# JBLanier/stratego_env

Hardware: AMD Instinct MI355X
Metric: env steps/sec (higher is better)
Workload: dtype u8

## Files before the change

stratego_env_amd/csrc/sgx_layout.h:

```cpp
#pragma once

namespace {

constexpr int OBS_CH = SGX_PO_OBS_CHANNELS;
constexpr int LUT_STRIDE = SGX_OBS_LUT_STRIDE;
constexpr int FOBS_CH = SGX_FO_OBS_CHANNELS;
constexpr int LUT_ROW_PITCH = 33, LUT_BLK = 673 , LUT_DWORDS = 2 * LUT_BLK + 2;
#ifndef SGX_WPB
#define SGX_WPB 8
#endif
#ifndef SGX_MIN_WAVES
#define SGX_MIN_WAVES 6
#endif
constexpr int QTAB_DWORDS = 2 * OBS_CH * 4, OBS_TAB_DWORDS = LUT_DWORDS + QTAB_DWORDS;
constexpr int FOBS_TAB_DWORDS = LUT_DWORDS + 2 * FOBS_CH * 4;
constexpr int NIB_ONE = 4, CODE_NONE = 0xFF, CODETAB_REC = 192, CODETAB_BYTES = 208;
constexpr int COMBAT_BYTES = 16 * 16;
enum { COMBAT_LOSE = 0, COMBAT_TIE = 1, COMBAT_WIN = 2, COMBAT_WIN_FLAG = 3 };
__host__ __device__ inline int combat_outcome(int att, int def) {
    if (att == 3  && def == 12 ) return COMBAT_WIN;
    if (att == 1  && def == 10 ) return COMBAT_WIN;
    if (def == 11 ) return COMBAT_WIN_FLAG;
    if (def == 12) return COMBAT_LOSE;
    if (att == def) return COMBAT_TIE;
// ... 168 lines not shown
    z ^= z >> 30; z *= 0xBF58476D1CE4E5B9ull;
    z ^= z >> 27; z *= 0x94D049BB133111EBull;
    z ^= z >> 31;
    return z;
}
__host__ __device__ inline uint64_t sgx_rng(uint64_t seed, uint64_t g, uint64_t j, uint32_t stream, uint32_t t) {
    uint64_t h = sm_fin(seed + 0x9E3779B97F4A7C15ull * (g + 1));
    uint64_t ctr = ((uint64_t)stream << 32) | t;
    return sm_fin(h ^ (j * 0xD1B54A32D192ED03ull + ctr * 0x8CB92BA72F3D8DD7ull + 0x2545F4914F6CDD1Dull));
}
__host__ __device__ inline uint32_t rng_below(uint64_t r, uint32_t n) { return (uint32_t)(((r >> 32) * (uint64_t)n) >> 32); }
enum { STREAM_SETUP = 0, STREAM_ACTION = 1, STREAM_SHUFFLE_P1 = 2, STREAM_SHUFFLE_P2 = 3, STREAM_POOL = 4, STREAM_DETERMINIZE = 5 };
__host__ __device__ inline int pool_index(uint64_t seed, uint64_t g, uint64_t j, int n_pool) {
    return (int)rng_below(sgx_rng(seed, g, j, STREAM_POOL, 0), (uint32_t)n_pool);
}
__host__ __device__ inline int pool_first_player(uint64_t seed, uint64_t g, uint64_t j, int pool_flags) {
    if (!(pool_flags & SGX_POOL_RANDOM_FIRST_PLAYER)) return 0;
    return rng_below(sgx_rng(seed, g, j, STREAM_POOL, 1), 2u) == 1u ? -1 : 1;
}

template <class G>
__device__ inline int4 *rec_scal(int8_t *boards, int rec_bytes, int64_t env) {
    return reinterpret_cast<int4 *>(boards + env * (int64_t)rec_bytes + G::SC_OFF);
}

template <class G, class KP>
__device__ inline int max_events_of(const KP &P) { return G::BIG ? (int)G::EVL_MAX : P.max_events; }

template <class G>
__device__ inline int uni(int x) {
    if constexpr (G::LPG == 64) return __builtin_amdgcn_readfirstlane(x);
    else return x;
}
template <class G>
__device__ inline unsigned long long gballot(bool pred) {
    const unsigned long long b = __ballot(pred);
    if constexpr (G::LPG == 64) return b;
    else return (b >> (__lane_id() & ~(G::LPG - 1))) & ((1ull << G::LPG) - 1ull);
}

template <int CTRL, int ROW_MASK = 0xF>
__device__ inline int dpp_or_zero(int x) { return __builtin_amdgcn_update_dpp(0, x, CTRL, ROW_MASK, 0xF, true); }
template <class G>
__device__ inline int gscan_incl(int x) {
    x += dpp_or_zero<0x111>(x);
    x += dpp_or_zero<0x112>(x);
    x += dpp_or_zero<0x114>(x);
    x += dpp_or_zero<0x118>(x);
    if constexpr (G::LPG >= 32) x += dpp_or_zero<0x142, 0xA>(x);
    if constexpr (G::LPG == 64) x += dpp_or_zero<0x143, 0xC>(x);
    return x;
}
template <class G>
__device__ inline int glane(int x, int l) {
    if constexpr (G::LPG == 64) return __builtin_amdgcn_readlane(x, __builtin_amdgcn_readfirstlane(l));
    else return __shfl(x, l, G::LPG);
}
__device__ inline int quad_sum(int x) {
    x += __builtin_amdgcn_update_dpp(0, x, 0xB1, 0xF, 0xF, true);
    x += __builtin_amdgcn_update_dpp(0, x, 0x4E, 0xF, 0xF, true);
    return x;
}

template <class KP>
__device__ inline int64_t group_of_block(const KP &P) {
    const int64_t nb = gridDim.x, b = blockIdx.x;
    const int x = (int)(b & 7);
    const int64_t i = b >> 3;
    if (P.map_mode == 0) {
        if (i >= P.xcd_count[x]) return (int64_t)1 << 40;
        return P.xcd_first[x] + i;
    }
    const int64_t per = nb >> 3;
    const int map_arg = P.map_arg;
    if (P.map_mode == 1) return b;
    if (P.map_mode == 2) { const int64_t s = map_arg; return (i / s) * (8 * s) + x * s + (i % s); }
    if (P.map_mode == 3) return x * per + (i + x * (int64_t)map_arg) % per;
    if (P.map_mode == 4) return x * per + (per - 1 - i);
    if (P.map_mode == 5) return x * per + ((x & 1) ? per - 1 - i : i);
    if (P.map_mode == 6) { const int64_t f = map_arg, sub = per / f; return x * per + (i % f) * sub + (i / f); }
    return x * per + i;
}

template <class G>
__device__ inline void wave_sync() {
    __builtin_amdgcn_fence(__ATOMIC_RELEASE, "wavefront");
    __builtin_amdgcn_wave_barrier();
    __builtin_amdgcn_fence(__ATOMIC_ACQUIRE, "wavefront");
}

struct PartialObs {
    static constexpr int NCH = OBS_CH;
    static constexpr bool CODES = true;
    static constexpr int OWN0 = 0, ENEMY0 = -1 , OWN_PO0 = 12, ENEMY_PO0 = 25, OBST = 38, REC0 = 39, CAP0 = 41,
                         STILL0 = 65;
};
struct FullObs {
    static constexpr int NCH = FOBS_CH;
    static constexpr bool CODES = true;
    static constexpr int OWN0 = 0, ENEMY0 = 12, OWN_PO0 = 24, ENEMY_PO0 = 37, OBST = 50, REC0 = 51, CAP0 = 53, STILL0 = 77;
};
struct OrigPartialObs {
    static constexpr int NCH = SGX_PO_OBS_CHANNELS_ORIGINAL;
    static constexpr bool CODES = false;
    static constexpr int REC0 = 4, CAP0 = 6;
    __device__ static inline int board(int ch, int qi) {
        if (ch == 0) return B_PIECES + qi;
        if (ch == 1) return B_PO + qi;
        if (ch == 2) return B_PO + (1 - qi);
        if (ch == 3) return B_OBST;
        if (ch == 4) return B_RECENT + qi;
        if (ch == 5) return B_RECENT + (1 - qi);
        if (ch < 30) return B_ZERO;
        if (ch == 30) return B_STILL + qi;
        return B_STILL + (1 - qi);
    }
    __device__ static inline int bias(int ch) { return (ch == 4 || ch == 5) ? 3 : 0; }
};
struct OrigFullObs {
    static constexpr int NCH = SGX_FO_OBS_CHANNELS_ORIGINAL;
    static constexpr bool CODES = false;
    static constexpr int REC0 = 3, CAP0 = 7;
    __device__ static inline int board(int ch, int qi) {
        if (ch == 0) return B_PIECES + qi;
        if (ch == 1) return B_PIECES + (1 - qi);
        if (ch == 2) return B_OBST;
        if (ch == 3) return B_RECENT + qi;
        if (ch == 4) return B_RECENT + (1 - qi);
        if (ch == 5) return B_PO + qi;
        if (ch == 6) return B_PO + (1 - qi);
        if (ch < 31) return B_ZERO;
        if (ch == 31) return B_STILL + qi;
        return B_STILL + (1 - qi);
    }
    __device__ static inline int bias(int ch) { return (ch == 3 || ch == 4) ? 3 : 0; }
};
template <int KIND>
struct ObsKind {
    static constexpr bool FULL = (KIND & 1) != 0, ORIG = (KIND & 2) != 0, NOOBS = (KIND & 8) != 0;
    static_assert(!NOOBS || KIND == 8, "the no-observation kind stands alone");
    static constexpr int NIB_CH = (ORIG || NOOBS) ? 0 : (FULL ? FOBS_CH : OBS_CH);
    using P = std::conditional_t<ORIG, OrigPartialObs, PartialObs>;
    using F = std::conditional_t<ORIG, OrigFullObs, FullObs>;
};

}
```

stratego_env_amd/csrc/sgx_step.h:

```cpp
#pragma once

namespace {

template <class G, int KIND>
constexpr int tmpl_bytes(bool full) { return ((G::RC * (full ? FOBS_CH : OBS_CH) + 1) / 2 + 15) & ~15; }
template <class G, int KIND>
constexpr int tmpl_lds_bytes(bool full) { return G::WIDE ? 0 : tmpl_bytes<G, KIND>(full); }
template <class G, int KIND>
constexpr int shared_table_bytes() {
    constexpr bool FULL = (KIND & 1) != 0, ORIG = (KIND & 2) != 0;
    if (ObsKind<KIND>::NOOBS) return 16;
    if (ORIG) return 4 * (OBS_TAB_DWORDS + (FULL ? FOBS_TAB_DWORDS : 0));
    return tmpl_lds_bytes<G, KIND>(false) + (FULL ? tmpl_lds_bytes<G, KIND>(true) : 0) + CODETAB_BYTES;
}

template <class G, int KIND, bool MAPPED = false>
constexpr int waves_per_simd() {
    constexpr int per_wg = G::WPB * G::GPW * (int)sizeof(Lds<G, ObsKind<KIND>::NIB_CH>) + shared_table_bytes<G, KIND>() + G::OBST_BYTES + COMBAT_BYTES;
    constexpr int wgs = (160 * 1024) / per_wg;
    constexpr int w = wgs * G::WPB / 4;
    constexpr int want = (G::HALF || (MAPPED && ObsKind<KIND>::NOOBS)) ? 6 : (G::RC <= 64 ? 8 : SGX_MIN_WAVES);
    return w > want ? want : (w < 1 ? 1 : w);
}

// ... 568 lines not shown
        const int na = kth_valid(L, (int)k, lane);
        if constexpr (PERSIST) {
            carry->na = na;
            if (lane == 0 && P.traj_act_log) P.traj_act_log[env + (int64_t)carry->slot * P.traj_out_envs] = na;
        }
        if (lane == 0 && (!PERSIST || last)) P.io.next_actions_dev[env] = na;
    }

    STAMP(7);
    bool dirty = applied || wrote_reset || (MAPPED && P.src_boards);
    if constexpr (PERSIST) {
        dirty = dirty || (!first && carry->dirty);
        carry->turn = turn; carry->flags = flags; carry->game_no = game_no; carry->max_turns = max_turns;
        carry->n_events = n_events; carry->rp0 = rp0; carry->rp1 = rp1; carry->dirty = dirty;
        if (!last) dirty = false;
    }
    if (dirty)
        write_record(L, rec_g, G::BIG ? (int)G::IMG_BYTES : P.rec_bytes, make_int4(turn, flags, max_turns, game_no), make_int4(n_events, rp0, rp1, 0), n_events, lane);
    STAMP(8);
#ifdef SGX_STAMPS
    asm volatile("s_waitcnt vmcnt(0)" ::: "memory");
    STAMP(9);
#endif
}

template <int R_, int C_, int KIND, bool MAPPED, int VAR = 0>
__device__ __forceinline__ void game_kernel_body(const KParams &P) {
    using G = Geo<R_, C_, VAR>;
    static_assert(VAR == 0 || (VAR == 2 && ObsKind<KIND>::NOOBS), "two games per wave: the no-observation kinds only");
    using PS = typename ObsKind<KIND>::P;
    using FS = typename ObsKind<KIND>::F;
    constexpr bool FULL = ObsKind<KIND>::FULL, ORIG = ObsKind<KIND>::ORIG;
    __shared__ Lds<G, ObsKind<KIND>::NIB_CH> LW[G::WPB * G::GPW];
    __shared__ alignas(16) uint8_t shared[shared_table_bytes<G, KIND>()];
    __shared__ alignas(16) uint8_t obst_s[G::OBST_BYTES + COMBAT_BYTES];
    const int lane = threadIdx.x & (G::LPG - 1), slot = threadIdx.x / G::LPG;
    const int64_t env = P.env_first + group_of_block(P) * (G::WPB * G::GPW) + slot;
    const GameInput in = load_game<G, MAPPED>(P, env, lane);
    const bool raw = (P.io.flags & SGX_STEP_RAW_OBS) != 0;
    if constexpr (ObsKind<KIND>::NOOBS) {
    } else if constexpr (ORIG) {
        float *lut_s = reinterpret_cast<float *>(shared);
        const f32x4 *lsrc = reinterpret_cast<const f32x4 *>(P.tab->lut[4 + (raw ? 2 : 0)]);
        for (int i = threadIdx.x; i < LUT_DWORDS / 4; i += 64 * G::WPB) reinterpret_cast<f32x4 *>(lut_s)[i] = lsrc[i];
        build_quad_table<G, PS>(reinterpret_cast<uint32_t *>(lut_s + LUT_DWORDS), threadIdx.x, 64 * G::WPB);
        if constexpr (FULL) {
            const f32x4 *fsrc = reinterpret_cast<const f32x4 *>(P.tab->lut[4 + (raw ? 2 : 0) + 1]);
            for (int i = threadIdx.x; i < LUT_DWORDS / 4; i += 64 * G::WPB) reinterpret_cast<f32x4 *>(lut_s + OBS_TAB_DWORDS)[i] = fsrc[i];
            build_quad_table<G, FS>(reinterpret_cast<uint32_t *>(lut_s + OBS_TAB_DWORDS + LUT_DWORDS), threadIdx.x, 64 * G::WPB);
        }
    } else {
        constexpr int NP = tmpl_lds_bytes<G, KIND>(false), NF = FULL ? tmpl_lds_bytes<G, KIND>(true) : 0;
        const int4 *tp = reinterpret_cast<const int4 *>(P.tab->tmpl[raw ? 2 : 0]);
        for (int i = threadIdx.x; i < NP / 16; i += 64 * G::WPB) reinterpret_cast<int4 *>(shared)[i] = tp[i];
        if constexpr (FULL) {
            const int4 *tf = reinterpret_cast<const int4 *>(P.tab->tmpl[(raw ? 2 : 0) + 1]);
            for (int i = threadIdx.x; i < NF / 16; i += 64 * G::WPB) reinterpret_cast<int4 *>(shared + NP)[i] = tf[i];
        }
        const int4 *ct = reinterpret_cast<const int4 *>(P.tab->codetab[raw ? 1 : 0]);
        for (int i = threadIdx.x; i < CODETAB_BYTES / 16; i += 64 * G::WPB) reinterpret_cast<int4 *>(shared + NP + NF)[i] = ct[i];
    }
    for (int i = threadIdx.x; i < G::S / 4; i += 64 * G::WPB) reinterpret_cast<int *>(obst_s)[i] = reinterpret_cast<const int *>(P.tab->obstacles)[i];
    for (int i = threadIdx.x; i < COMBAT_BYTES / 4; i += 64 * G::WPB)
        reinterpret_cast<int *>(obst_s + G::OBST_BYTES)[i] = reinterpret_cast<const int *>(P.tab->combat)[i];
    __syncthreads();
    if (env < P.n_envs) env_step<R_, C_, KIND, MAPPED, false, VAR>(P, LW[slot], shared, obst_s, env, lane, in);
}

template <int R_, int C_, int KIND, bool MAPPED = false, int VAR = 0>
__global__ __launch_bounds__((64 * Geo<R_, C_, VAR>::WPB), (waves_per_simd<Geo<R_, C_, VAR>, KIND, MAPPED>())) void step_kernel(const KParams P) {
    game_kernel_body<R_, C_, KIND, MAPPED, VAR>(P);
}
template <int R_, int C_, int KIND, bool MAPPED = false, int VAR = 0>
__global__ __launch_bounds__((64 * Geo<R_, C_, VAR>::WPB), (waves_per_simd<Geo<R_, C_, VAR>, KIND, MAPPED>())) void observe_kernel(const KParams P) {
    game_kernel_body<R_, C_, KIND, MAPPED, VAR>(P);
}

constexpr int WSTEPS_MAX_SETS = 8;
struct WaveStepsParams {
    KParams k;
    int32_t n_steps, n_sets, first_set;
    int32_t strided;
    int32_t barrier;
    int64_t obs_slot_bytes, fobs_slot_bytes, mask_slot_bytes;
    float *const *obs_tab, *const *fobs_tab;
    uint8_t *const *mask_tab;
    float *obs[WSTEPS_MAX_SETS], *fobs[WSTEPS_MAX_SETS];
    uint8_t *mask[WSTEPS_MAX_SETS];
};
template <class SPP>
__device__ __forceinline__ void steps_outputs_of(const SPP sp, const int set, StepCarry &carry) {
    if (sp->strided == 2) {
        carry.obs = table_entry(sp->obs_tab, set);
        carry.fobs = table_entry(sp->fobs_tab, set);
        carry.mask = table_entry(sp->mask_tab, set);
    } else if (sp->strided) {
        carry.obs = reinterpret_cast<float *>(reinterpret_cast<char *>(sp->obs[0]) + (int64_t)set * sp->obs_slot_bytes);
        carry.fobs = reinterpret_cast<float *>(reinterpret_cast<char *>(sp->fobs[0]) + (int64_t)set * sp->fobs_slot_bytes);
        carry.mask = sp->mask[0] + (int64_t)set * sp->mask_slot_bytes;
    } else {
        carry.obs = sp->obs[set];
        carry.fobs = sp->fobs[set];
        carry.mask = sp->mask[set];
    }
    carry.slot = set;
}
template <class G, int KIND>
constexpr int steps_waves_per_simd() {
    constexpr int w = waves_per_simd<G, KIND, false>();
    return (G::RC <= 64 && G::RC % 4 != 0 && !ObsKind<KIND>::NOOBS && w > 6) ? 6 : w;
}
struct WaveStepsParamsPool {
    WaveStepsParams w;
    PoolParams pool;
};
__device__ __forceinline__ const SGX_KERNARG WaveStepsParams *wsp_of(const SGX_KERNARG WaveStepsParams *p) { return p; }
__device__ __forceinline__ const SGX_KERNARG WaveStepsParams *wsp_of(const SGX_KERNARG WaveStepsParamsPool *p) { return &p->w; }
template <int R_, int C_, int KIND, int VAR, class SPT = WaveStepsParamsPool>
__device__ __forceinline__ void steps_body(const SPT &SP) {
    constexpr bool POOL = true;
    using G = Geo<R_, C_, VAR>;
    static_assert(VAR == 0 || (VAR == 2 && ObsKind<KIND>::NOOBS), "two games per wave: the no-observation kinds only");
    using PS = typename ObsKind<KIND>::P;
    using FS = typename ObsKind<KIND>::F;
    constexpr bool FULL = ObsKind<KIND>::FULL, ORIG = ObsKind<KIND>::ORIG;
#if defined(__HIP_DEVICE_COMPILE__)
    const SGX_KERNARG SPT *top = (const SGX_KERNARG SPT *)__builtin_amdgcn_kernarg_segment_ptr();
#else
    const SPT *top = &SP;
#endif
    const SGX_KERNARG WaveStepsParams *spp = wsp_of(top);
    const SGX_KERNARG KParams &P = spp->k;
    __shared__ Lds<G, ObsKind<KIND>::NIB_CH> LW[G::WPB * G::GPW];
    __shared__ alignas(16) uint8_t shared[shared_table_bytes<G, KIND>()];
    __shared__ alignas(16) uint8_t obst_s[G::OBST_BYTES + COMBAT_BYTES];
    const int lane = threadIdx.x & (G::LPG - 1), slot = threadIdx.x / G::LPG;
    const int64_t env = P.env_first + group_of_block(P) * (G::WPB * G::GPW) + slot;
    const GameInput in = load_game<G, false>(P, env, lane);
    const bool raw = (P.io.flags & SGX_STEP_RAW_OBS) != 0;
    if constexpr (ObsKind<KIND>::NOOBS) {
    } else if constexpr (ORIG) {
        float *lut_s = reinterpret_cast<float *>(shared);
        const f32x4 *lsrc = reinterpret_cast<const f32x4 *>(P.tab->lut[4 + (raw ? 2 : 0)]);
        for (int i = threadIdx.x; i < LUT_DWORDS / 4; i += 64 * G::WPB) reinterpret_cast<f32x4 *>(lut_s)[i] = lsrc[i];
        build_quad_table<G, PS>(reinterpret_cast<uint32_t *>(lut_s + LUT_DWORDS), threadIdx.x, 64 * G::WPB);
        if constexpr (FULL) {
            const f32x4 *fsrc = reinterpret_cast<const f32x4 *>(P.tab->lut[4 + (raw ? 2 : 0) + 1]);
            for (int i = threadIdx.x; i < LUT_DWORDS / 4; i += 64 * G::WPB) reinterpret_cast<f32x4 *>(lut_s + OBS_TAB_DWORDS)[i] = fsrc[i];
            build_quad_table<G, FS>(reinterpret_cast<uint32_t *>(lut_s + OBS_TAB_DWORDS + LUT_DWORDS), threadIdx.x, 64 * G::WPB);
        }
    } else {
        constexpr int NP = tmpl_lds_bytes<G, KIND>(false), NF = FULL ? tmpl_lds_bytes<G, KIND>(true) : 0;
        const int4 *tp = reinterpret_cast<const int4 *>(P.tab->tmpl[raw ? 2 : 0]);
        for (int i = threadIdx.x; i < NP / 16; i += 64 * G::WPB) reinterpret_cast<int4 *>(shared)[i] = tp[i];
        if constexpr (FULL) {
            const int4 *tf = reinterpret_cast<const int4 *>(P.tab->tmpl[(raw ? 2 : 0) + 1]);
            for (int i = threadIdx.x; i < NF / 16; i += 64 * G::WPB) reinterpret_cast<int4 *>(shared + NP)[i] = tf[i];
        }
        const int4 *ct = reinterpret_cast<const int4 *>(P.tab->codetab[raw ? 1 : 0]);
        for (int i = threadIdx.x; i < CODETAB_BYTES / 16; i += 64 * G::WPB) reinterpret_cast<int4 *>(shared + NP + NF)[i] = ct[i];
    }
    for (int i = threadIdx.x; i < G::S / 4; i += 64 * G::WPB) reinterpret_cast<int *>(obst_s)[i] = reinterpret_cast<const int *>(P.tab->obstacles)[i];
    for (int i = threadIdx.x; i < COMBAT_BYTES / 4; i += 64 * G::WPB)
        reinterpret_cast<int *>(obst_s + G::OBST_BYTES)[i] = reinterpret_cast<const int *>(P.tab->combat)[i];
    __syncthreads();
    if (env >= P.n_envs) return;
    int set = spp->first_set;
    const int n_steps = spp->n_steps;
    if constexpr (POOL) {
        StepCarryPool carry{};
        for (int t = 0; t < n_steps; ++t) {
            const SGX_KERNARG SPT *tp = top;
            int lane_t = lane, slot_t = slot;
            asm volatile("" : "+s"(tp), "+v"(lane_t), "+v"(slot_t));
            const SGX_KERNARG WaveStepsParams *sp = wsp_of(tp);
            if (t && sp->barrier) __builtin_amdgcn_s_barrier();
            steps_outputs_of(sp, set, carry);
            carry.first = t == 0;
            env_step<R_, C_, KIND, false, false, VAR, 3, true>(sp->k, LW[slot_t], shared, obst_s, env, lane_t, in, nullptr, nullptr, &carry, t == n_steps - 1, &tp->pool);
            set = set + 1 == sp->n_sets ? 0 : set + 1;
        }
    }
}
template <int R_, int C_, int KIND, int VAR = 0>
__global__ __launch_bounds__((64 * Geo<R_, C_, VAR>::WPB), (steps_waves_per_simd<Geo<R_, C_, VAR>, KIND>())) void steps_kernel(const WaveStepsParams SP) {
    using G = Geo<R_, C_, VAR>;
    static_assert(VAR == 0 || (VAR == 2 && ObsKind<KIND>::NOOBS), "two games per wave: the no-observation kinds only");
    using PS = typename ObsKind<KIND>::P;
    using FS = typename ObsKind<KIND>::F;
    constexpr bool FULL = ObsKind<KIND>::FULL, ORIG = ObsKind<KIND>::ORIG;
#if defined(__HIP_DEVICE_COMPILE__)
    const SGX_KERNARG WaveStepsParams *spp = (const SGX_KERNARG WaveStepsParams *)__builtin_amdgcn_kernarg_segment_ptr();
#else
    const WaveStepsParams *spp = &SP;
#endif
    const SGX_KERNARG KParams &P = spp->k;
    __shared__ Lds<G, ObsKind<KIND>::NIB_CH> LW[G::WPB * G::GPW];
    __shared__ alignas(16) uint8_t shared[shared_table_bytes<G, KIND>()];
    __shared__ alignas(16) uint8_t obst_s[G::OBST_BYTES + COMBAT_BYTES];
    const int lane = threadIdx.x & (G::LPG - 1), slot = threadIdx.x / G::LPG;
    const int64_t env = P.env_first + group_of_block(P) * (G::WPB * G::GPW) + slot;
    const GameInput in = load_game<G, false>(P, env, lane);
    const bool raw = (P.io.flags & SGX_STEP_RAW_OBS) != 0;
    if constexpr (ObsKind<KIND>::NOOBS) {
    } else if constexpr (ORIG) {
        float *lut_s = reinterpret_cast<float *>(shared);
        const f32x4 *lsrc = reinterpret_cast<const f32x4 *>(P.tab->lut[4 + (raw ? 2 : 0)]);
        for (int i = threadIdx.x; i < LUT_DWORDS / 4; i += 64 * G::WPB) reinterpret_cast<f32x4 *>(lut_s)[i] = lsrc[i];
        build_quad_table<G, PS>(reinterpret_cast<uint32_t *>(lut_s + LUT_DWORDS), threadIdx.x, 64 * G::WPB);
        if constexpr (FULL) {
            const f32x4 *fsrc = reinterpret_cast<const f32x4 *>(P.tab->lut[4 + (raw ? 2 : 0) + 1]);
            for (int i = threadIdx.x; i < LUT_DWORDS / 4; i += 64 * G::WPB) reinterpret_cast<f32x4 *>(lut_s + OBS_TAB_DWORDS)[i] = fsrc[i];
            build_quad_table<G, FS>(reinterpret_cast<uint32_t *>(lut_s + OBS_TAB_DWORDS + LUT_DWORDS), threadIdx.x, 64 * G::WPB);
        }
    } else {
        constexpr int NP = tmpl_lds_bytes<G, KIND>(false), NF = FULL ? tmpl_lds_bytes<G, KIND>(true) : 0;
        const int4 *tp = reinterpret_cast<const int4 *>(P.tab->tmpl[raw ? 2 : 0]);
        for (int i = threadIdx.x; i < NP / 16; i += 64 * G::WPB) reinterpret_cast<int4 *>(shared)[i] = tp[i];
        if constexpr (FULL) {
            const int4 *tf = reinterpret_cast<const int4 *>(P.tab->tmpl[(raw ? 2 : 0) + 1]);
            for (int i = threadIdx.x; i < NF / 16; i += 64 * G::WPB) reinterpret_cast<int4 *>(shared + NP)[i] = tf[i];
        }
        const int4 *ct = reinterpret_cast<const int4 *>(P.tab->codetab[raw ? 1 : 0]);
        for (int i = threadIdx.x; i < CODETAB_BYTES / 16; i += 64 * G::WPB) reinterpret_cast<int4 *>(shared + NP + NF)[i] = ct[i];
    }
    for (int i = threadIdx.x; i < G::S / 4; i += 64 * G::WPB) reinterpret_cast<int *>(obst_s)[i] = reinterpret_cast<const int *>(P.tab->obstacles)[i];
    for (int i = threadIdx.x; i < COMBAT_BYTES / 4; i += 64 * G::WPB)
        reinterpret_cast<int *>(obst_s + G::OBST_BYTES)[i] = reinterpret_cast<const int *>(P.tab->combat)[i];
    __syncthreads();
    if (env >= P.n_envs) return;
    StepCarry carry{0, 0, 0, 0, 0, 0, 0, 0, false, nullptr, nullptr, nullptr, 0};
    int set = spp->first_set;
    const int n_steps = spp->n_steps;
    {
        steps_outputs_of(spp, set, carry);
        env_step<R_, C_, KIND, false, false, VAR, 1>(P, LW[slot], shared, obst_s, env, lane, in, nullptr, nullptr, &carry, n_steps == 1);
        set = set + 1 == spp->n_sets ? 0 : set + 1;
    }
    for (int t = 1; t < n_steps; ++t) {
        const SGX_KERNARG WaveStepsParams *sp = spp;
        int lane_t = lane, slot_t = slot;
        asm volatile("" : "+s"(sp), "+v"(lane_t), "+v"(slot_t));
        if (sp->barrier) __builtin_amdgcn_s_barrier();
        steps_outputs_of(sp, set, carry);
#ifdef SGX_MUTANT_SKIP_STORE
        if (t == 3) carry.obs = nullptr;
#endif
        env_step<R_, C_, KIND, false, false, VAR, 2>(sp->k, LW[slot_t], shared, obst_s, env, lane_t, in, nullptr, nullptr, &carry, t == n_steps - 1);
        set = set + 1 == sp->n_sets ? 0 : set + 1;
    }
}
template <int R_, int C_, int KIND, int VAR = 0>
__global__ __launch_bounds__((64 * Geo<R_, C_, VAR>::WPB), (steps_waves_per_simd<Geo<R_, C_, VAR>, KIND>())) void steps_kernel_pool(const WaveStepsParamsPool SP) {
    steps_body<R_, C_, KIND, VAR>(SP);
}

constexpr int SINGLE_WAVES = 8;
template <int R_, int C_, int KIND, bool POOL>
__device__ __forceinline__ void single_body(const KParams &P, uint32_t *__restrict__ done_count, uint32_t *__restrict__ flag_host, const uint32_t seq,
                                            const PoolParams *pp = nullptr) {
    using G = Geo<R_, C_>;
    using PS = typename ObsKind<KIND>::P;
    using FS = typename ObsKind<KIND>::F;
    constexpr bool FULL = ObsKind<KIND>::FULL;
    static_assert(!ObsKind<KIND>::ORIG && G::LPG == 64 && !G::WIDE && G::RC % 4 == 0, "single_kernel: 'extended' kinds, 4-aligned one-game-per-wave boards");
    constexpr int NT = 64 * SINGLE_WAVES, RC = G::RC;
    __shared__ Lds<G, ObsKind<KIND>::NIB_CH> L;
    __shared__ alignas(16) uint8_t shared[shared_table_bytes<G, KIND>()];
    __shared__ alignas(16) uint8_t obst_s[G::OBST_BYTES + COMBAT_BYTES];
    __shared__ StepOut so;
    const int tid = threadIdx.x, lane = tid & 63, wave = tid >> 6;
    const int64_t env = P.env_first + blockIdx.x;
    GameInput in{};
    if (wave == 0) in = load_game<G, false>(P, env, lane);
    const bool raw = (P.io.flags & SGX_STEP_RAW_OBS) != 0;
    constexpr int NP = tmpl_lds_bytes<G, KIND>(false), NF = FULL ? tmpl_lds_bytes<G, KIND>(true) : 0;
    {
        const int4 *tp = reinterpret_cast<const int4 *>(P.tab->tmpl[raw ? 2 : 0]);
        for (int i = tid; i < NP / 16; i += NT) reinterpret_cast<int4 *>(shared)[i] = tp[i];
        if constexpr (FULL) {
            const int4 *tf = reinterpret_cast<const int4 *>(P.tab->tmpl[(raw ? 2 : 0) + 1]);
            for (int i = tid; i < NF / 16; i += NT) reinterpret_cast<int4 *>(shared + NP)[i] = tf[i];
        }
        const int4 *ct = reinterpret_cast<const int4 *>(P.tab->codetab[raw ? 1 : 0]);
        for (int i = tid; i < CODETAB_BYTES / 16; i += NT) reinterpret_cast<int4 *>(shared + NP + NF)[i] = ct[i];
        for (int i = tid; i < G::S / 4; i += NT) reinterpret_cast<int *>(obst_s)[i] = reinterpret_cast<const int *>(P.tab->obstacles)[i];
        for (int i = tid; i < COMBAT_BYTES / 4; i += NT) reinterpret_cast<int *>(obst_s + G::OBST_BYTES)[i] = reinterpret_cast<const int *>(P.tab->combat)[i];
    }
    __syncthreads();
    if (wave == 0) env_step<R_, C_, KIND, false, true, 0, 0, POOL>(P, L, shared, obst_s, env, lane, in, nullptr, &so, nullptr, true, pp);
    __syncthreads();
    if (P.io.mask_dev) emit_mask<G, NT>(L, P.io.mask_dev + env * (int64_t)G::NA, tid);
    const uint8_t *codetab = shared + NP + NF;
    auto render_all = [&](auto spec, bool full, float *dst) {
        using Spec = decltype(spec);
        if (wave == 0) {
            const int n_unc = build_codes<G, Spec>(L, full ? shared + NP : shared, codetab, P.tab->lut[(raw ? 2 : 0) + (full ? 1 : 0)], so.qi,
                                                   so.n_events, so.rp0, so.rp1, lane, P.piece_counts, raw, P.multi_ev != 0);
            if (lane == 0) so.n_unc = n_unc;
        }
        __syncthreads();
        const int n_unc = so.n_unc;
        if (n_unc == 0) emit_codes<G, Spec, false, false, NT>(L, dst, tid);
        else {
            emit_codes<G, Spec, true, false, NT>(L, dst, tid);
            if (wave == 0) patch_uncoded<G, Spec>(L, dst, n_unc, lane);
        }
        __syncthreads();
    };
    if (P.io.obs_dev) render_all(PS{}, false, P.io.obs_dev + env * (int64_t)(RC * PS::NCH));
    if constexpr (FULL)
        if (P.io.fobs_dev) render_all(FS{}, true, P.io.fobs_dev + env * (int64_t)(RC * FS::NCH));
// ... 24 lines not shown
```

stratego_env_amd/csrc/stratego_mi355x.hip:

```cpp
#include <hip/hip_runtime.h>
#include <type_traits>
#include <stdint.h>
#include <stdio.h>
#include <stdlib.h>
#include <sched.h>
#include <time.h>
#include <string.h>
#include <string>
#include <vector>

#include "stratego_mi355x.h"

#define SGX_API extern "C" __attribute__((visibility("default")))

namespace {

thread_local std::string g_last_error;

int fail(int code, const char *fmt, const char *detail = "") {
    char buf[512];
    snprintf(buf, sizeof(buf), fmt, detail);
    g_last_error = buf;
    return code;
}

#define HIP_TRY(expr)                                                                        \
    do {                                                                                     \
        hipError_t e_ = (expr);                                                              \
        if (e_ != hipSuccess) return fail(SGX_EDEVICE, #expr ": %s", hipGetErrorString(e_)); \
    } while (0)

struct DeviceGuard {
    int prev = -1;
    bool restore = false;
    hipError_t err = hipSuccess;
    explicit DeviceGuard(int dev) {
        err = hipGetDevice(&prev);
        if (err == hipSuccess && prev != dev) {
            err = hipSetDevice(dev);
            restore = err == hipSuccess;
        }
    }
    ~DeviceGuard() {
        if (restore) (void)hipSetDevice(prev);
    }
    DeviceGuard(const DeviceGuard &) = delete;
    DeviceGuard &operator=(const DeviceGuard &) = delete;
};
#define SGX_ON_DEVICE(dev)                                                                                      \
    DeviceGuard device_guard_(dev);                                                                             \
    if (device_guard_.err != hipSuccess) return fail(SGX_EDEVICE, "selecting the handle's device: %s", hipGetErrorString(device_guard_.err))

#ifndef SGX_BUILD_ID
#define SGX_BUILD_ID "unknown"
#endif
const char g_build_id[] = "SGX_BUILD_ID=" SGX_BUILD_ID;

}

#include "sgx_layout.h"
#include "sgx_obs.h"
#include "sgx_mask.h"
#include "sgx_setup.h"
#include "sgx_step.h"
#include "sgx_lane.h"
#include "sgx_lane_kernel.h"
#include "sgx_aux_kernels.h"
#include "sgx_choose.h"
#include "sgx_mem.h"


struct sgx_env {
    sgx_config cfg;
    int64_t n_envs;
    int device;
    uint64_t seed;
    int64_t env_id_offset;
    int8_t *boards;
    DevTables *tab;
    uint8_t *setups;
    int64_t n_setups;
    int rec_bytes;
    int sc_off;
    int max_events;
    int K;
    unsigned long long *stamps;
    int map_mode, map_arg;
    int xcd_skew;
    int xcd_explicit;
    int32_t xcd_w[8];
    int nt_mode;
    int lane_mode;
    float placement_target_us;
    hipStream_t chain_stream[SGX_MAX_CHAINS];
    hipEvent_t chain_fork, chain_join[SGX_MAX_CHAINS];
    uint32_t *sync_flag_host, *sync_flag_dev, *sync_count;
    uint32_t sync_seq;
    int no_single;
    uint8_t *san_flags;
    int32_t *redo_list;
    int general_states;
    int no_multi_step;
    int multi_step_attr;
    int multi_step_attr_pool;
    int last_kind;
    int multi_step_wave;
    int steps_barrier;
    int half_wave;
    void **ring_tab_dev, **ring_tab_host;
    int ring_tab_cap, ring_tab_n;
    hipEvent_t ring_tab_ev;
    hipStream_t ring_tab_stream;
    int8_t *pool;
    int64_t n_pool;
    int pool_flags;
    int32_t *start_index;
};

namespace {

#ifdef SGX_ONLY_EXTRA
#define SGX_BUILTIN_GEOMETRIES(X, A)
#else
#define SGX_BUILTIN_GEOMETRIES(X, A) X(A, 10, 10) X(A, 15, 15) X(A, 8, 8) X(A, 6, 6) X(A, 5, 5) X(A, 4, 4) X(A, 3, 4)
#endif
#ifdef SGX_EXTRA_R
#define SGX_EXTRA_GEOMETRY(X, A) X(A, SGX_EXTRA_R, SGX_EXTRA_C)
static_assert(SGX_EXTRA_R >= 3 && SGX_EXTRA_C >= 3 && SGX_EXTRA_R * SGX_EXTRA_C <= SGX_MAX_CELLS, "SGX_EXTRA_R x SGX_EXTRA_C out of range");
#else
#define SGX_EXTRA_GEOMETRY(X, A)
#endif
#define SGX_ALL_GEOMETRIES(X, A) SGX_BUILTIN_GEOMETRIES(X, A) SGX_EXTRA_GEOMETRY(X, A)

bool supported_geometry(int r, int c) {
#define SGX_MATCH(A, R, C) if (r == (R) && c == (C)) return true;
    SGX_ALL_GEOMETRIES(SGX_MATCH, _)
#undef SGX_MATCH
    return false;
}

template <int N> using int_c = std::integral_constant<int, N>;
template <bool B> using bool_c = std::integral_constant<bool, B>;

template <class F>
int for_geometry(const sgx_env *h, F &&f) {
    const int r = h->cfg.rows, c = h->cfg.cols;
#define SGX_DISPATCH_ONE(A, R, C) if (r == (R) && c == (C)) { f(int_c<(R)>(), int_c<(C)>()); return SGX_OK; }
    SGX_ALL_GEOMETRIES(SGX_DISPATCH_ONE, _)
#undef SGX_DISPATCH_ONE
    return fail(SGX_EINVAL, "unsupported board size%s");
}

int compact_capacity(const sgx_env *h) { return h->max_events + 4; }
int compact_obs_stride(const sgx_env *h) {
    const int nib = ((h->cfg.rows * h->cfg.cols * OBS_CH + 1) / 2 + 15) & ~15;
    return (nib + 16 + 8 * compact_capacity(h) + 127) & ~127;
}
int mask_words(const sgx_env *h) {
    const int na = h->cfg.rows * h->cfg.cols * h->K;
    return (((na + 31) / 32 + 1) + 3) & ~3;
}

KParams make_params(const sgx_env *h) {
    KParams p;
    memset(&p, 0, sizeof(p));
    p.boards = h->boards;
    p.tab = h->tab;
    p.setups = h->setups;
    p.n_setups = (int32_t)h->n_setups;
    p.max_turns = h->cfg.max_turns;
    p.usable_rows = h->cfg.usable_rows;
    for (int i = 0; i < 12; ++i) p.piece_counts[i] = h->cfg.piece_counts[i];
    p.rec_bytes = h->rec_bytes;
    p.max_events = h->max_events;
    for (int i = 0; i < 12; ++i)
        if (h->cfg.piece_counts[i] > EV_COUNT_MAX) p.multi_ev = 1;
    p.compact_stride = compact_obs_stride(h);
    p.n_envs = h->n_envs;
    p.seed = h->seed;
    p.env_id_offset = h->env_id_offset;
#ifdef SGX_STAMPS
    p.stamps = h->stamps;
#endif
    return p;
}

PoolParams make_pool_params(const sgx_env *h, int64_t index_off = 0) {
    PoolParams pp;
    pp.pool = h->pool;
    pp.n_pool = (int32_t)h->n_pool;
// ... 114 lines not shown
                }
            }
        }
        uint8_t *ct = tab->codetab[raw];
        memset(ct, CODE_NONE, CODETAB_BYTES);
        for (int t = 0; t < 12; ++t)
            for (int v = 0; v < LUT_STRIDE; ++v) {
                const float f = dense[0][(41 + t) * LUT_STRIDE + v];
                if (f != dense[0][(53 + t) * LUT_STRIDE + v] || f != dense[1][(53 + t) * LUT_STRIDE + v] || f != dense[1][(65 + t) * LUT_STRIDE + v])
                    return fail(SGX_EINVAL, "captured-count channels of one piece type are normalised differently%s");
                ct[16 * t + v] = (uint8_t)float_code(f);
            }
        for (int v = 0; v < 5; ++v) {
            const float f = dense[0][39 * LUT_STRIDE + v];
            if (f != dense[0][40 * LUT_STRIDE + v] || f != dense[1][51 * LUT_STRIDE + v] || f != dense[1][52 * LUT_STRIDE + v])
                return fail(SGX_EINVAL, "recent-move channels are normalised differently%s");
            ct[CODETAB_REC + v] = (uint8_t)float_code(f);
        }
    }
    return SGX_OK;
}

SGX_API int sgx_build_obs_lut(const sgx_config *cfg, float *lut) {
    if (int rc = check_cfg(cfg)) return rc;
    if (!lut) return fail(SGX_EINVAL, "lut is NULL%s");
    build_lut(cfg, false, lut);
    return SGX_OK;
}

SGX_API int sgx_build_full_obs_lut(const sgx_config *cfg, float *lut) {
    if (int rc = check_cfg(cfg)) return rc;
    if (!lut) return fail(SGX_EINVAL, "lut is NULL%s");
    build_lut(cfg, true, lut);
    return SGX_OK;
}

SGX_API int sgx_build_original_obs_lut(const sgx_config *cfg, int32_t full, float *lut) {
    if (int rc = check_cfg(cfg)) return rc;
    if (!lut) return fail(SGX_EINVAL, "lut is NULL%s");
    build_lut(cfg, full != 0, lut, false, true);
    return SGX_OK;
}

SGX_API int sgx_create(const sgx_config *cfg, int64_t n_envs, int device, uint64_t seed, int64_t env_id_offset, sgx_env **out) {
    if (!out) return fail(SGX_EINVAL, "out is NULL%s");
    *out = nullptr;
    if (int rc = check_cfg(cfg)) return rc;
    if (!supported_geometry(cfg->rows, cfg->cols))
        return fail(SGX_EINVAL, "board size not compiled into this library (built in: 10x10, 15x15, 8x8, 6x6, 5x5, 4x4, 3x4; any other size: "
                                "build the same sources with -DSGX_EXTRA_R=<rows> -DSGX_EXTRA_C=<cols>, stratego_env_amd/build.py build_geometry)%s");
    if (n_envs <= 0 || n_envs > (int64_t)1 << 30) return fail(SGX_EINVAL, "n_envs out of range%s");
    int ndev = 0;
    hipError_t e = hipGetDeviceCount(&ndev);
    if (e != hipSuccess || ndev <= 0) return fail(SGX_EDEVICE, "no HIP device available: %s", hipGetErrorString(e));
    if (device < 0 || device >= ndev) return fail(SGX_EINVAL, "device index out of range%s");
    SGX_ON_DEVICE(device);
    sgx_env *h = new sgx_env();
    memset(h, 0, sizeof(*h));
    h->cfg = *cfg;
    h->n_envs = n_envs;
    h->device = device;
    h->seed = seed;
    h->env_id_offset = env_id_offset;
    h->nt_mode = -1;
    if (const char *e = getenv("SGX_NT")) {
        if (!strcmp(e, "0")) h->nt_mode = 0;
        else if (!strcmp(e, "1")) h->nt_mode = 1;
    }
    h->lane_mode = -1;
    h->general_states = 1;
    if (const char *e = getenv("SGX_GENERAL_STATES")) h->general_states = atoi(e);
    if (const char *e = getenv("SGX_LANE")) { if (!strcmp(e, "0")) h->lane_mode = 0; else if (!strcmp(e, "1")) h->lane_mode = 1; }
    h->xcd_skew = -1;
    if (const char *e = getenv("SGX_XCD_SKEW")) { if (strcmp(e, "auto")) h->xcd_skew = atoi(e); }
    if (h->xcd_skew > 900) h->xcd_skew = 900;
    if (const char *e = getenv("SGX_NO_SINGLE")) h->no_single = atoi(e);
    if (const char *e = getenv("SGX_MULTI_STEP")) h->no_multi_step = !strcmp(e, "0");
    h->multi_step_wave = 1;
    if (const char *e = getenv("SGX_MULTI_STEP_WAVE")) h->multi_step_wave = strcmp(e, "0") != 0;
    h->half_wave = 1;
    if (const char *e = getenv("SGX_HALF_WAVE")) h->half_wave = strcmp(e, "0") != 0;
    h->steps_barrier = -1;
    if (const char *e = getenv("SGX_STEPS_BARRIER")) h->steps_barrier = !strcmp(e, "0") ? 0 : !strcmp(e, "1") ? 1 : -1;
    if (const char *e = getenv("SGX_MAP")) { h->map_mode = atoi(e); if (const char *c = strchr(e, ',')) h->map_arg = atoi(c + 1); }
    const int rc_cells = cfg->rows * cfg->cols;
    {
        int pieces = 0;
        for (int i = 0; i < 12; ++i) pieces += cfg->piece_counts[i];
        if (cfg->capture_capacity > pieces) pieces = cfg->capture_capacity;
        h->max_events = 2 * pieces;
        if (h->max_events > rc_cells) h->max_events = rc_cells;
        const int st_off = (STORED_BOARDS * ((rc_cells + 3) & ~3) + 15) & ~15, sb = (((rc_cells + 7) / 8) + 15) & ~15;
        const int sc_off = st_off + 2 * sb;
        h->sc_off = sc_off;
        h->rec_bytes = (sc_off + 32 + (rc_cells > 256 ? 4 : 2) * h->max_events + 127) & ~127;
    }
    h->K = 2 * (cfg->rows - 1) + 2 * (cfg->cols - 1) + 1;
    DevTables host_tab;
    memset(&host_tab, 0, sizeof(host_tab));
    {
        float dense[FOBS_CH * LUT_STRIDE];
        for (int k = 0; k < 8; ++k) {
            const bool original = (k & 4) != 0, raw = (k & 2) != 0, full = (k & 1) != 0;
            build_lut(cfg, full, dense, raw, original);
            for (int ch = 0; ch < lut_channels(full, original); ++ch)
                for (int i = 0; i < LUT_STRIDE; ++i) host_tab.lut[k][lut_row(ch) + i] = dense[ch * LUT_STRIDE + i];
        }
    }
    memcpy(host_tab.obstacles, cfg->obstacles, rc_cells);
    if (int rc = build_code_tables(cfg, &host_tab)) { delete h; return rc; }
    for (int a = 0; a < 16; ++a)
        for (int d = 0; d < 16; ++d) host_tab.combat[16 * a + d] = (uint8_t)combat_outcome(a, d);
    if (hipMalloc((void **)&h->boards, (size_t)n_envs * h->rec_bytes) != hipSuccess ||
        hipMalloc((void **)&h->tab, sizeof(DevTables)) != hipSuccess) {
        sgx_destroy(h);
        return fail(SGX_ENOMEM, "device allocation failed%s");
    }
#define HIP_TRY_OR_DESTROY(expr)                                                             \
    do {                                                                                     \
        hipError_t e_ = (expr);                                                              \
        if (e_ != hipSuccess) { sgx_destroy(h); return fail(SGX_EDEVICE, #expr ": %s", hipGetErrorString(e_)); } \
    } while (0)
    HIP_TRY_OR_DESTROY(hipMemset(h->boards, 0, (size_t)n_envs * h->rec_bytes));
    HIP_TRY_OR_DESTROY(hipMemcpy(h->tab, &host_tab, sizeof(DevTables), hipMemcpyHostToDevice));
#ifdef SGX_STAMPS
    HIP_TRY_OR_DESTROY(hipMalloc((void **)&h->stamps, (size_t)n_envs * 16 * sizeof(unsigned long long)));
    HIP_TRY_OR_DESTROY(hipMemset(h->stamps, 0, (size_t)n_envs * 16 * sizeof(unsigned long long)));
#endif
    init_scal_kernel<<<(unsigned)((n_envs + 255) / 256), 256>>>(h->boards, h->rec_bytes, h->sc_off, n_envs, cfg->max_turns);
    HIP_TRY_OR_DESTROY(hipGetLastError());
    HIP_TRY_OR_DESTROY(hipDeviceSynchronize());
#undef HIP_TRY_OR_DESTROY
    *out = h;
    return SGX_OK;
}

SGX_API int sgx_destroy(sgx_env *h) {
    if (!h) return SGX_OK;
    DeviceGuard device_guard_(h->device);
    (void)hipDeviceSynchronize();
    if (h->boards) (void)hipFree(h->boards);
    if (h->tab) (void)hipFree(h->tab);
    if (h->setups) (void)hipFree(h->setups);
    if (h->pool) (void)hipFree(h->pool);
    if (h->stamps) (void)hipFree(h->stamps);
    for (int c = 0; c < SGX_MAX_CHAINS; ++c) {
        if (h->chain_stream[c]) (void)hipStreamDestroy(h->chain_stream[c]);
        if (h->chain_join[c]) (void)hipEventDestroy(h->chain_join[c]);
    }
    if (h->chain_fork) (void)hipEventDestroy(h->chain_fork);
    if (h->sync_flag_host) (void)hipHostFree(h->sync_flag_host);
    if (h->sync_count) (void)hipFree(h->sync_count);
    if (h->san_flags) (void)hipFree(h->san_flags);
    if (h->redo_list) (void)hipFree(h->redo_list);
    if (h->ring_tab_dev) (void)hipFree(h->ring_tab_dev);
    if (h->ring_tab_host) (void)hipHostFree(h->ring_tab_host);
    if (h->ring_tab_ev) (void)hipEventDestroy(h->ring_tab_ev);
    delete h;
    return SGX_OK;
}

SGX_API int sgx_set_nt_stores(sgx_env *h, int32_t mode) {
    if (!h || mode < -1 || mode > 1) return fail(SGX_EINVAL, "sgx_set_nt_stores: mode must be -1 (auto), 0 or 1%s");
    h->nt_mode = mode;
    return SGX_OK;
}
// ... 337 lines not shown
    }
    for (int32_t k = 0; k < sets.n_sets; ++k) {
        KParams pk = p;
        pk.io = sets.ios[k];
        const bool full = pk.io.fobs_dev || pk.io.final_fobs_dev, original = (pk.io.flags & SGX_STEP_ORIGINAL_CHANNELS) != 0;
        if (!pk.io.obs_dev || !lane_eligible(h, pk, full, original, true)) return false;
    }
    return true;
}

static bool wave_steps_ok(const sgx_env *h, const KParams &p, const OutSets &sets) {
    const sgx_step_io &io0 = p.io;
    if (!h->multi_step_wave || h->map_mode != 0) return false;
    if (io0.flags & (SGX_STEP_ACTIONS_1D | SGX_STEP_ACTIONS_POSITIONS | SGX_STEP_MASK_1D | SGX_STEP_MASK_STATE_COORDS | SGX_STEP_ORIGINAL_CHANNELS)) return false;
    const bool compact = (io0.flags & (SGX_STEP_COMPACT_OBS | SGX_STEP_COMPACT_MASK)) != 0;
    const bool full = io0.fobs_dev || io0.final_fobs_dev;
    const bool no_obs = !io0.obs_dev && !io0.fobs_dev && !io0.final_obs_dev && !io0.final_fobs_dev && !compact;
    auto misaligned = [](const sgx_step_io &io) { return ((reinterpret_cast<uintptr_t>(io.obs_dev) | reinterpret_cast<uintptr_t>(io.mask_dev)) & 15) != 0; };
    if (compact && (full || io0.final_obs_dev)) return false;
    if (compact && misaligned(io0)) return false;
    if (no_obs && h->cfg.rows * h->cfg.cols <= 12 && lane_eligible(h, p, false, false)) return false;
    if (sets.strided) return !(compact && ((sets.obs_b | sets.mask_b) & 15));
    for (int32_t k = 0; k < sets.n_sets; ++k) {
        const sgx_step_io &io = sets.ios[k];
        if (io.final_obs_dev != io0.final_obs_dev || io.final_fobs_dev != io0.final_fobs_dev || (io.obs_dev == nullptr) != (io0.obs_dev == nullptr) ||
            (io.fobs_dev == nullptr) != (io0.fobs_dev == nullptr) || (io.mask_dev == nullptr) != (io0.mask_dev == nullptr)) return false;
        if (compact && misaligned(io)) return false;
    }
    return true;
}

static bool sets_share_results(const OutSets &sets, const sgx_step_io &io0) {
    if (sets.strided) return true;
    for (int32_t k = 0; k < sets.n_sets; ++k) {
        const sgx_step_io &io = sets.ios[k];
        if (io.reward_dev != io0.reward_dev || io.done_dev != io0.done_dev || io.player_dev != io0.player_dev || io.invalid_action_dev != io0.invalid_action_dev ||
            io.ending_invalid_dev != io0.ending_invalid_dev) return false;
    }
    return true;
}

static int steps_launch(sgx_env *h, StepsParams &sp, KParams &p, const int32_t *w, hipStream_t stream, bool *ok) {
    *ok = false;
    return for_geometry(h, [&](auto r, auto c) {
        constexpr int R = decltype(r)::value, C = decltype(c)::value;
        if constexpr (lane_geometry<Geo<R, C>>()) {
            const unsigned grid = grid_for(p, 64, w);
            const size_t dyn = 2 * 64 * (size_t)(p.rec_bytes + 16);
            if (dyn + sizeof(StepsLds<Geo<R, C>>) > 64 * 1024 && !h->multi_step_attr) {
                if (hipFuncSetAttribute(reinterpret_cast<const void *>(&lane_steps_kernel<R, C>), hipFuncAttributeMaxDynamicSharedMemorySize, (int)dyn) != hipSuccess) {
                    (void)hipGetLastError();
                    h->no_multi_step = 1;
                    return;
                }
                h->multi_step_attr = 1;
            }
            sp.k = p;
            if (h->pool) {
                if (dyn + sizeof(StepsLds<Geo<R, C>>) > 64 * 1024 && !h->multi_step_attr_pool) {
                    if (hipFuncSetAttribute(reinterpret_cast<const void *>(&lane_steps_kernel_pool<R, C>), hipFuncAttributeMaxDynamicSharedMemorySize, (int)dyn) != hipSuccess) {
                        (void)hipGetLastError();
                        h->no_multi_step = 1;
                        return;
                    }
                    h->multi_step_attr_pool = 1;
                }
                lane_steps_kernel_pool<R, C><<<grid, 64 * (1 + KSTEP_EMITTERS), dyn, stream>>>(sp, make_pool_params(h));
            } else
                lane_steps_kernel<R, C><<<grid, 64 * (1 + KSTEP_EMITTERS), dyn, stream>>>(sp);
            *ok = true;
        }
    });
}

static int steps_launch(sgx_env *h, WaveStepsParams &sp, KParams &p, const int32_t *w, hipStream_t stream, bool *ok) {
    const sgx_step_io &io = p.io;
    const bool compact = (io.flags & (SGX_STEP_COMPACT_OBS | SGX_STEP_COMPACT_MASK)) != 0;
    const bool no_obs = !io.obs_dev && !io.fobs_dev && !io.final_obs_dev && !io.final_fobs_dev && !compact;
    const int kind = compact ? 4 : no_obs ? 8 : (io.fobs_dev || io.final_fobs_dev) ? 1 : 0;
    const int cells = h->cfg.rows * h->cfg.cols;
    const bool pays = (kind == 0 || kind == 1) && cells >= 36 && cells <= 225 && sp.n_sets >= (cells == 100 ? WSTEPS_MAX_SETS + 1 : 16);
    const bool want_barrier = h->steps_barrier > 0 || (h->steps_barrier < 0 && pays);
    *ok = true;
    return for_geometry(h, [&](auto r, auto c) {
        constexpr int R = decltype(r)::value, C = decltype(c)::value;
        auto launch = [&](auto kind_c) {
            constexpr int KIND = decltype(kind_c)::value;
            with_half_wave<R, C, KIND>(h, [&](auto var) {
                constexpr int VAR = decltype(var)::value;
                using G = Geo<R, C, VAR>;
                const unsigned grid = geo_grid<G>(p, w);
                sp.k = p;
                sp.barrier = want_barrier && (p.n_envs - p.env_first) % (G::WPB * G::GPW) == 0;
                if (h->pool) steps_kernel_pool<R, C, KIND, VAR><<<grid, 64 * G::WPB, 0, stream>>>(WaveStepsParamsPool{sp, make_pool_params(h)});
                else steps_kernel<R, C, KIND, VAR><<<grid, 64 * G::WPB, 0, stream>>>(sp);
            });
        };
        if (kind == 0) launch(int_c<0>());
        else if (kind == 1) launch(int_c<1>());
        else if (kind == 4) launch(int_c<4>());
        else launch(int_c<8>());
    });
}

template <class SP>
static int multi_step(sgx_env *h, const KParams &p_in, const OutSets &sets, int32_t first, int32_t n_steps, void *stream, bool *launched) {
    constexpr bool lane = std::is_same<SP, StepsParams>::value;
    *launched = false;
    const int32_t n_sets = sets.n_sets;
    KParams p = p_in;
    p.mode = 0;
    p.io = sets.ios[sets.strided ? 0 : first];
    if (n_steps < 2 || h->no_multi_step || !(lane ? lane_steps_ok(h, p, sets) : wave_steps_ok(h, p, sets)) || !sets_share_results(sets, p.io)) return SGX_OK;
    if (int rc = check_step_io(h, p)) return rc;
    SP sp;
    memset(&sp, 0, sizeof(sp));
    sp.n_sets = n_sets;
    if (sets.strided) {
        sp.strided = 1;
        sp.obs_slot_bytes = sets.obs_b; sp.mask_slot_bytes = sets.mask_b;
        sp.obs[0] = p.io.obs_dev; sp.mask[0] = p.io.mask_dev;
        if constexpr (!lane) { sp.fobs_slot_bytes = sets.fobs_b; sp.fobs[0] = p.io.fobs_dev; }
    } else if (n_sets > (int32_t)std::extent<decltype(sp.obs)>::value) {
        void **tab = nullptr;
        if (int rc = upload_ring_table(h, sets, (hipStream_t)stream, &tab)) return rc;
        sp.strided = 2;
        sp.obs_tab = reinterpret_cast<float *const *>(tab);
        sp.mask_tab = reinterpret_cast<uint8_t *const *>(tab + 2 * n_sets);
        if constexpr (!lane) sp.fobs_tab = reinterpret_cast<float *const *>(tab + n_sets);
    } else
        for (int32_t k = 0; k < n_sets; ++k) {
            sp.obs[k] = sets.ios[k].obs_dev; sp.mask[k] = sets.ios[k].mask_dev;
            if constexpr (!lane) sp.fobs[k] = sets.ios[k].fobs_dev;
        }
    int32_t w[8];
    launch_setup(h, p, n_sets, w);
    for (int32_t done = 0; done < n_steps; ) {
        const int32_t now = n_steps - done > SGX_STEPS_MAX_PER_LAUNCH ? SGX_STEPS_MAX_PER_LAUNCH : n_steps - done;
        const int32_t set = (int32_t)(((int64_t)first + done) % n_sets);
        if (now < 2) {
            if (int rc = launch_set_step(h, p_in, sets, set, stream)) return rc;
        } else {
            sp.n_steps = now; sp.first_set = set;
            bool ok = false;
            if (int rc = steps_launch(h, sp, p, w, (hipStream_t)stream, &ok)) return rc;
            if (!ok) {
                if (done == 0) return SGX_OK;
                return fail(SGX_EDEVICE, "lane_steps_kernel became unavailable in the middle of a call%s");
            }
            HIP_TRY(hipGetLastError());
        }
        done += now;
    }
    *launched = true;
    h->last_kind = lane ? SGX_LAUNCH_MULTI_STEP : SGX_LAUNCH_MULTI_STEP_WAVE;
    return SGX_OK;
}

static int multi_steps(sgx_env *h, const KParams &p, const OutSets &sets, int32_t first, int32_t n_steps, void *stream, bool *launched) {
    if (int rc = multi_step<StepsParams>(h, p, sets, first, n_steps, stream, launched)) return rc;
    if (*launched) return SGX_OK;
    return multi_step<WaveStepsParams>(h, p, sets, first, n_steps, stream, launched);
}

static int play_steps(sgx_env *h, const KParams &p, const OutSets &sets, int32_t first, int32_t n_steps, void *stream) {
    bool launched = false;
    if (int rc = multi_steps(h, p, sets, first, n_steps, stream, &launched)) return rc;
    for (int32_t i = 0; i < n_steps && !launched; ++i)
        if (int rc = launch_set_step(h, p, sets, (int32_t)(((int64_t)first + i) % sets.n_sets), stream)) return rc;
    return SGX_OK;
}

static int launch_step(sgx_env *h, const KParams &p_in, void *stream, int ring_sets, int64_t start_index_off, bool allow_pool) {
    KParams p = p_in;
    if (int rc = check_step_io(h, p)) return rc;
    int32_t w[8];
    launch_setup(h, p, ring_sets, w);
    const hipStream_t st = (hipStream_t)stream;
    const bool full = p.io.fobs_dev || p.io.final_fobs_dev, original = (p.io.flags & SGX_STEP_ORIGINAL_CHANNELS) != 0;
    const bool compact = (p.io.flags & (SGX_STEP_COMPACT_OBS | SGX_STEP_COMPACT_MASK)) != 0;
    const bool pool = allow_pool && h->pool != nullptr && p.mode == 0;
    const PoolParams pool_params = make_pool_params(h, start_index_off);
    if (compact) {
        if (full || original || p.io.final_obs_dev || p.src_boards || (p.io.flags & (SGX_STEP_MASK_1D | SGX_STEP_MASK_STATE_COORDS)))
            return fail(SGX_EINVAL, "compact outputs come with the 67-channel partial observation and the perspective mask only (no fobs / final_obs / original channels / state-coordinate masks)%s");
// ... 874 lines not shown
```

Baseline: 260.6 million.

## Use persistent resident workgroups for the 10x10 multi-step kernel

For 10x10 boards without half-wave packing, the multi-step kernel launches only as many workgroups as can be resident at once, sized from an occupancy query and capped per XCD. Each workgroup loops over game groups with a stride and reuses the LDS tables it loaded once. The aim is to avoid repeated per-block setup of the shared observation and combat tables, and the scheduling cost of many short blocks. The trade-off is possible load imbalance and reliance on the occupancy estimate, and it is disabled when the barrier path or pool mode is active.

```diff
diff --git a/stratego_env_amd/csrc/sgx_layout.h b/stratego_env_amd/csrc/sgx_layout.h
--- a/stratego_env_amd/csrc/sgx_layout.h
+++ b/stratego_env_amd/csrc/sgx_layout.h
@@ -274,6 +274,13 @@
     return x * per + i;
 }
 
+template <class KP>
+__device__ inline void groups_of_block(const KP &P, int64_t &group, int64_t &end) {
+    const int x = (int)(blockIdx.x & 7);
+    group = P.xcd_first[x] + (int64_t)(blockIdx.x >> 3);
+    end = P.xcd_first[x] + (int64_t)P.xcd_count[x];
+}
+
 template <class G>
 __device__ inline void wave_sync() {
     __builtin_amdgcn_fence(__ATOMIC_RELEASE, "wavefront");
diff --git a/stratego_env_amd/csrc/sgx_step.h b/stratego_env_amd/csrc/sgx_step.h
--- a/stratego_env_amd/csrc/sgx_step.h
+++ b/stratego_env_amd/csrc/sgx_step.h
@@ -674,6 +674,7 @@
     int32_t n_steps, n_sets, first_set;
     int32_t strided;
     int32_t barrier;
+    int32_t stride;
     int64_t obs_slot_bytes, fobs_slot_bytes, mask_slot_bytes;
     float *const *obs_tab, *const *fobs_tab;
     uint8_t *const *mask_tab;
@@ -702,6 +703,8 @@
     constexpr int w = waves_per_simd<G, KIND, false>();
     return (G::RC <= 64 && G::RC % 4 != 0 && !ObsKind<KIND>::NOOBS && w > 6) ? 6 : w;
 }
+template <int R_, int C_, int KIND, int VAR>
+constexpr bool steps_resident() { return R_ == 10 && C_ == 10 && VAR == 0; }
 struct WaveStepsParamsPool {
     WaveStepsParams w;
     PoolParams pool;
@@ -791,8 +794,9 @@
     __shared__ alignas(16) uint8_t shared[shared_table_bytes<G, KIND>()];
     __shared__ alignas(16) uint8_t obst_s[G::OBST_BYTES + COMBAT_BYTES];
     const int lane = threadIdx.x & (G::LPG - 1), slot = threadIdx.x / G::LPG;
-    const int64_t env = P.env_first + group_of_block(P) * (G::WPB * G::GPW) + slot;
-    const GameInput in = load_game<G, false>(P, env, lane);
+    constexpr bool RESIDENT = steps_resident<R_, C_, KIND, VAR>();
+    const int64_t env = RESIDENT ? 0 : P.env_first + group_of_block(P) * (G::WPB * G::GPW) + slot;
+    const GameInput in = RESIDENT ? GameInput{} : load_game<G, false>(P, env, lane);
     const bool raw = (P.io.flags & SGX_STEP_RAW_OBS) != 0;
     if constexpr (ObsKind<KIND>::NOOBS) {
     } else if constexpr (ORIG) {
@@ -820,6 +824,38 @@
     for (int i = threadIdx.x; i < COMBAT_BYTES / 4; i += 64 * G::WPB)
         reinterpret_cast<int *>(obst_s + G::OBST_BYTES)[i] = reinterpret_cast<const int *>(P.tab->combat)[i];
     __syncthreads();
+    if constexpr (RESIDENT) {
+        int64_t group, end;
+        groups_of_block(P, group, end);
+        for (; group < end; group += spp->stride) {
+            const SGX_KERNARG WaveStepsParams *sg = spp;
+            int lane_g = lane, slot_g = slot;
+            asm volatile("" : "+s"(sg), "+v"(lane_g), "+v"(slot_g));
+            const SGX_KERNARG KParams &Pg = sg->k;
+            const int64_t env_g = Pg.env_first + group * (G::WPB * G::GPW) + slot_g;
+            if (env_g >= Pg.n_envs) break;
+            const GameInput in_g = load_game<G, false>(Pg, env_g, lane_g);
+            StepCarry carry{0, 0, 0, 0, 0, 0, 0, 0, false, nullptr, nullptr, nullptr, 0};
+            int set = sg->first_set;
+            const int n_steps = sg->n_steps;
+            steps_outputs_of(sg, set, carry);
+            env_step<R_, C_, KIND, false, false, VAR, 1>(Pg, LW[slot_g], shared, obst_s, env_g, lane_g, in_g, nullptr, nullptr, &carry, n_steps == 1);
+            set = set + 1 == sg->n_sets ? 0 : set + 1;
+            for (int t = 1; t < n_steps; ++t) {
+                const SGX_KERNARG WaveStepsParams *sp = sg;
+                int lane_t = lane_g, slot_t = slot_g;
+                asm volatile("" : "+s"(sp), "+v"(lane_t), "+v"(slot_t));
+                if (sp->barrier) __builtin_amdgcn_s_barrier();
+                steps_outputs_of(sp, set, carry);
+#ifdef SGX_MUTANT_SKIP_STORE
+                if (t == 3) carry.obs = nullptr;
+#endif
+                env_step<R_, C_, KIND, false, false, VAR, 2>(sp->k, LW[slot_t], shared, obst_s, env_g, lane_t, in_g, nullptr, nullptr, &carry, t == n_steps - 1);
+                set = set + 1 == sp->n_sets ? 0 : set + 1;
+            }
+        }
+        return;
+    }
     if (env >= P.n_envs) return;
     StepCarry carry{0, 0, 0, 0, 0, 0, 0, 0, false, nullptr, nullptr, nullptr, 0};
     int set = spp->first_set;
diff --git a/stratego_env_amd/csrc/stratego_mi355x.hip b/stratego_env_amd/csrc/stratego_mi355x.hip
--- a/stratego_env_amd/csrc/stratego_mi355x.hip
+++ b/stratego_env_amd/csrc/stratego_mi355x.hip
@@ -106,6 +106,8 @@
     int last_kind;
     int multi_step_wave;
     int steps_barrier;
+    int steps_resident;
+    int resident_slots[4];
     int half_wave;
     void **ring_tab_dev, **ring_tab_host;
     int ring_tab_cap, ring_tab_n;
@@ -386,6 +388,8 @@
     if (const char *e = getenv("SGX_HALF_WAVE")) h->half_wave = strcmp(e, "0") != 0;
     h->steps_barrier = -1;
     if (const char *e = getenv("SGX_STEPS_BARRIER")) h->steps_barrier = !strcmp(e, "0") ? 0 : !strcmp(e, "1") ? 1 : -1;
+    h->steps_resident = -1;
+    if (const char *e = getenv("SGX_STEPS_RESIDENT")) { if (strcmp(e, "auto")) h->steps_resident = atoi(e) < 0 ? -1 : atoi(e); }
     if (const char *e = getenv("SGX_MAP")) { h->map_mode = atoi(e); if (const char *c = strchr(e, ',')) h->map_arg = atoi(c + 1); }
     const int rc_cells = cfg->rows * cfg->cols;
     {
@@ -889,16 +893,37 @@
     const bool pays = (kind == 0 || kind == 1) && cells >= 36 && cells <= 225 && sp.n_sets >= (cells == 100 ? WSTEPS_MAX_SETS + 1 : 16);
     const bool want_barrier = h->steps_barrier > 0 || (h->steps_barrier < 0 && pays);
     *ok = true;
-    return for_geometry(h, [&](auto r, auto c) {
+    hipError_t slots_err = hipSuccess;
+    const int rc = for_geometry(h, [&](auto r, auto c) {
         constexpr int R = decltype(r)::value, C = decltype(c)::value;
         auto launch = [&](auto kind_c) {
             constexpr int KIND = decltype(kind_c)::value;
             with_half_wave<R, C, KIND>(h, [&](auto var) {
                 constexpr int VAR = decltype(var)::value;
                 using G = Geo<R, C, VAR>;
-                const unsigned grid = geo_grid<G>(p, w);
+                unsigned grid = geo_grid<G>(p, w);
                 sp.k = p;
                 sp.barrier = want_barrier && (p.n_envs - p.env_first) % (G::WPB * G::GPW) == 0;
+                if constexpr (steps_resident<R, C, KIND, VAR>()) {
+                    if (!h->pool && !sp.barrier && h->steps_resident != 0) {
+                        int slots = h->steps_resident;
+                        if (slots < 0) {
+                            int &known = h->resident_slots[KIND == 0 ? 0 : KIND == 1 ? 1 : KIND == 4 ? 2 : 3];
+                            if (!known) {
+                                int per_cu = 0, cus = 0;
+                                slots_err = hipOccupancyMaxActiveBlocksPerMultiprocessor(&per_cu, reinterpret_cast<const void *>(&steps_kernel<R, C, KIND, VAR>), 64 * G::WPB, 0);
+                                if (slots_err == hipSuccess) slots_err = hipDeviceGetAttribute(&cus, hipDeviceAttributeMultiprocessorCount, h->device);
+                                if (slots_err != hipSuccess) return;
+                                constexpr int promised = steps_waves_per_simd<G, KIND>() * 4 / G::WPB;
+                                if (per_cu > promised) per_cu = promised;
+                                known = per_cu * cus / 8 > 0 ? per_cu * cus / 8 : 1;
+                            }
+                            slots = known;
+                        }
+                        if (grid / 8 > (unsigned)slots) grid = 8 * (unsigned)slots;
+                    }
+                }
+                sp.stride = (int32_t)(grid / 8);
                 if (h->pool) steps_kernel_pool<R, C, KIND, VAR><<<grid, 64 * G::WPB, 0, stream>>>(WaveStepsParamsPool{sp, make_pool_params(h)});
                 else steps_kernel<R, C, KIND, VAR><<<grid, 64 * G::WPB, 0, stream>>>(sp);
             });
@@ -908,6 +933,8 @@
         else if (kind == 4) launch(int_c<4>());
         else launch(int_c<8>());
     });
+    if (slots_err != hipSuccess) return fail(SGX_EDEVICE, "steps_kernel: asking how many workgroups are resident: %s", hipGetErrorString(slots_err));
+    return rc;
 }
 
 template <class SP>
```

Result: slower. 236.1 million (-9.4%).
